# OpenMatchmaking/microservice-matchmaking

Measured on NVIDIA H100. Metric: matches/sec, higher is better.
Workload: dtype int32/u64

## Files before the change

microservice-matchmaking_b200/csrc/mm_common.cuh:

```cuda
#pragma once
#include <cuda_runtime.h>
#include <stdint.h>

#include "../../include/mm_engine.h"

namespace mm {

constexpr int kBlock = 512;
constexpr uint32_t kTile = 2048;
constexpr uint32_t kMaxRows = 2048;
constexpr uint32_t kMaxStages = 4;
constexpr uint32_t kTileBytes = kTile * (8 + 2);
constexpr uint32_t kMaxSegs = MM_MAX_GROUPS * MM_MAX_MODES;
constexpr uint32_t kChunkHist = 256;
constexpr uint32_t kFastBins = 255;
constexpr uint64_t kEmptyKey = 0xFFFFFFFFFFFFFFFFull;
constexpr uint64_t kTombKey = 0xFFFFFFFFFFFFFFFEull;
constexpr uint64_t kFreeVal = 0xFFFFFFFFFFFFFFFFull;
constexpr uint64_t kPending = 0x8000000000000000ull;
constexpr uint32_t kGenMask = 0x7FFFFFFFu;

struct PoolView {
  uint64_t* id;
  int32_t* rating;
  uint8_t* mode;
  uint8_t* tsize;
  uint32_t* ts;
  uint16_t* bin;
  uint32_t* seq;
};
struct PoolMeta {
  uint32_t* fill;
  uint32_t* chunk_tab;
  uint32_t* bump;
  uint32_t* tot;
  uint32_t* chist;
  uint32_t max_ch;
};

struct BinMap {
  const uint16_t* lut;
  int32_t key_lo;
  uint32_t KR;
  uint32_t stride;
  uint32_t K;
};

struct SegInfo {
  uint32_t n;
  uint32_t n_lobbies;
  uint32_t member_base;
  uint32_t lobby_base;
  uint32_t left_base;
  uint32_t new_chunk;
  uint32_t n_left;
  uint32_t reserved;
};

struct TickCtr {
  uint32_t gbar;
  uint32_t done;
  uint32_t n_lobbies, n_matched, n_alive, n_dead, n_resid;
  uint32_t n_tiles;
  uint32_t heavy;
  uint32_t chist_bad;
  unsigned long long t[12];
};

struct Geo {
  uint32_t T0[kMaxSegs + 1];
  uint32_t NT, tpr, n_segs, max_rows;
};

struct ActiveView {
  unsigned long long* kv;
  uint64_t mask;
  uint64_t dcap;
  __device__ __forceinline__ bool on() const { return mask != 0 || dcap != 0; }
  __device__ __forceinline__ unsigned long long* key(uint64_t h) const { return kv + 2 * h; }
  __device__ __forceinline__ unsigned long long* val(uint64_t h) const { return dcap ? kv + h : kv + 2 * h + 1; }
};

__device__ __forceinline__ uint64_t hash64(uint64_t x) {
  x ^= x >> 33; x *= 0xFF51AFD7ED558CCDull; x ^= x >> 33; x *= 0xC4CEB9FE1A85EC53ull; x ^= x >> 33;
  return x;
}
__device__ __forceinline__ uint64_t act_find(const ActiveView& a, uint64_t pid) {
  if (a.dcap) return pid < a.dcap ? pid : ~0ull;
  if (pid >= kTombKey) return ~0ull;
  uint64_t h = hash64(pid) & a.mask;
  for (uint64_t probe = 0; probe <= a.mask; ++probe) {
    const unsigned long long k = *a.key(h);
    if (k == pid) return h;
    if (k == kEmptyKey) return ~0ull;
    h = (h + 1) & a.mask;
  }
  return ~0ull;
}

__device__ __forceinline__ uint64_t policy_evict_first() {
  uint64_t p;
  asm volatile("createpolicy.fractional.L2::evict_first.b64 %0, 1.0;" : "=l"(p));
  return p;
}
__device__ __forceinline__ uint64_t policy_evict_last() {
  uint64_t p;
  asm volatile("createpolicy.fractional.L2::evict_last.b64 %0, 1.0;" : "=l"(p));
  return p;
}
__device__ __forceinline__ void st_hint_u64(uint64_t* a, uint64_t v, uint64_t pol) {
  asm volatile("st.global.L2::cache_hint.u64 [%0], %1, %2;" ::"l"(a), "l"(v), "l"(pol) : "memory");
}

__device__ __forceinline__ uint32_t smem_u32(const void* p) { return (uint32_t)__cvta_generic_to_shared(p); }
__device__ __forceinline__ void mbar_init(uint64_t* bar, uint32_t count) {
  asm volatile("mbarrier.init.shared::cta.b64 [%0], %1;" ::"r"(smem_u32(bar)), "r"(count) : "memory");
}
__device__ __forceinline__ void mbar_fence_init() { asm volatile("fence.mbarrier_init.release.cluster;" ::: "memory"); }
__device__ __forceinline__ void mbar_expect_tx(uint64_t* bar, uint32_t bytes) {
// ... 169 lines not shown
```

microservice-matchmaking_b200/csrc/mm_engine.cu:

```cuda
#include <cuda_runtime.h>

#include <algorithm>
#include <cstdio>
#include <cstdlib>
#include <cstring>
#include <mutex>
#include <new>
#include <vector>

#include "mm_kernels.cuh"

using namespace mm;

namespace {

struct Pool {
  PoolView v{};
  PoolMeta m{};
  uint32_t n = 0;
};

struct Table {
  unsigned long long* kv = nullptr;
};

}

struct mm_engine {
  mm_config cfg{};
  std::mutex mu;
  int device = 0;
  int n_sms = 0;
  size_t smem_optin = 0, smem_sm = 0;
  cudaStream_t stream = nullptr;
  bool own_stream = true;
  cudaStream_t copy_stream = nullptr;
  cudaEvent_t ev_copy = nullptr;
  cudaStream_t d2h_stream = nullptr;
  bool async_results = false, results_pending = false;
  bool last_packed = false;
  cudaEvent_t ev[5]{};
  char last_err[512] = {0};

  int32_t key_lo = 0;
  uint32_t KR = 0, stride = 0, K = 0, Kp = 0;
  uint32_t n_segs = 0;
  uint32_t n_cut = 0;
  uint16_t* d_part_cut = nullptr;
  uint32_t* d_cut_lp_lo = nullptr;
  uint16_t* d_lut = nullptr;
  uint8_t* d_grp_lut = nullptr;
  uint8_t* d_mode_tsize = nullptr;
  uint32_t* d_seg_bin_lo = nullptr;
  uint32_t* d_seg_L = nullptr;
  uint16_t* d_bin_seg = nullptr;
  uint32_t min_L = 1;
  uint32_t max_nb = 1;

  uint32_t capacity = 0;
  uint32_t n_chunks = 0;
  Pool pool[2];
  int cur = 0;
  uint32_t gen = 1;
  uint32_t seq_next = 0;
  Pool snap;
  uint32_t snap_gen = 0, snap_seq = 0;
  bool has_snap = false;

  bool use_active = true, dense_ids = false;
  uint64_t hcap = 0;
  Table tab[2];
  int tcur = 0;
  uint64_t n_active = 0, n_tomb = 0;

  uint32_t R = 0;
  uint32_t helpers = 0;
  int rows_per_sm = 2;
  int rank_impl = 3;
  uint32_t place_stages = 0;
  int fused_ok = 0;
  int tick_impl = 1;
  size_t tick_smem = 0;
  uint32_t *d_M = nullptr, *d_P = nullptr;
  uint32_t *d_outbase = nullptr, *d_binlim = nullptr;
  uint16_t* d_bin_key = nullptr;
// ... 436 lines not shown
  const uint32_t rows = tick_rows(e);
  k_place<512><<<rows, 512, place_smem_bytes(e->max_nb, e->place_stages), e->stream>>>(place_args(e, want_seq),
                                                                                  e->pool[e->cur].m.fill, e->n_segs);
  CK(cudaEventRecord(e->ev[3], e->stream));
  if (e->pool[e->cur ^ 1].m.chist)
    CK(cudaMemsetAsync(e->pool[e->cur ^ 1].m.chist, 0, (size_t)e->n_chunks * kChunkHist * 4, e->stream));
  k_epilogue<512><<<std::max<uint32_t>(1, std::min<uint32_t>((uint32_t)e->n_sms, 2 * rows)), 512, 0, e->stream>>>(epi_args(e, want_seq, true));
  CK(cudaGetLastError());
  CK(cudaEventRecord(e->ev[4], e->stream));
  CK(cudaMemcpyAsync(e->h_ctr, e->d_ctr, sizeof(TickCtr), cudaMemcpyDeviceToHost, e->stream));
  CK(cudaStreamSynchronize(e->stream));
  return MM_OK;
}

bool use_fused(const mm_engine* e) { return e->tick_impl == 1 && e->fused_ok; }

int tick_fused(mm_engine* e, bool want_seq) {
  TickArgs a{};
  const uint32_t rows = tick_rows(e);
  const uint32_t helpers = rows >= 64 ? std::min(32u, e->helpers + (e->R - rows)) : (rows > 1 ? 1u : 0u);
  a.src = e->pool[e->cur].v;
  a.R = rows;
  a.M = e->d_M;
  a.P = e->d_P;
  e->ctr_idx ^= 1;
  e->d_ctr = e->d_ctr2 + e->ctr_idx;
  a.tail = tail_args(e);
  a.place = place_args(e, want_seq);
  a.epi = epi_args(e, want_seq, want_seq || helpers == 0);
  a.next_ctr = e->d_ctr2 + (e->ctr_idx ^ 1);
  CK(cudaEventRecord(e->ev[0], e->stream));
  void* params[] = {&a};
  CK(cudaLaunchCooperativeKernel((const void*)k_tick<512>, dim3(rows + helpers), dim3(512), params, e->tick_smem, e->stream));
  CK(cudaEventRecord(e->ev[4], e->stream));
  CK(cudaMemcpyAsync(e->h_ctr, e->d_ctr, sizeof(TickCtr), cudaMemcpyDeviceToHost, e->stream));
  CK(cudaStreamSynchronize(e->stream));
  return MM_OK;
}

int tick_commit(mm_engine* e, uint32_t n, mm_tick_stats* stats) {
  const TickCtr& c = *e->h_ctr;
  mm_tick_stats st{};
  st.pool_before = n; st.n_lobbies = c.n_lobbies; st.n_matched = c.n_matched; st.n_residual = c.n_resid;
  st.n_dead = c.n_dead; st.n_launches = 4;
  float ms = 0;
  CK(cudaEventElapsedTime(&ms, e->ev[0], e->ev[4]));
  st.device_us = ms * 1000.f;
  if (e->last_fused) {
    st.n_launches = 1;
    st.hist_us = (float)(c.t[1] - c.t[0]) * 1e-3f;
    st.scan_us = (float)(c.t[2] - c.t[1]) * 1e-3f;
    st.place_us = (float)(c.t[3] - c.t[2]) * 1e-3f;
    st.epilogue_us = (float)(c.t[6] - c.t[3]) * 1e-3f;
    if (std::getenv("MM_TRACE"))
      std::fprintf(stderr, "[mm] t0=0 rows_p1_done=%.1f tail_done=%.1f bar1=%.1f place_start=%.1f rows_place_done=%.1f bar2=%.1f end=%.1f us\n",
                   (c.t[8] - c.t[0]) * 1e-3, (c.t[5] - c.t[0]) * 1e-3, (c.t[1] - c.t[0]) * 1e-3, (c.t[2] - c.t[0]) * 1e-3,
                   (c.t[10] - c.t[0]) * 1e-3, (c.t[3] - c.t[0]) * 1e-3, (c.t[6] - c.t[0]) * 1e-3);
  } else {
    CK(cudaEventElapsedTime(&ms, e->ev[0], e->ev[1]));
    st.hist_us = ms * 1000.f;
    CK(cudaEventElapsedTime(&ms, e->ev[1], e->ev[2]));
    st.scan_us = ms * 1000.f;
    CK(cudaEventElapsedTime(&ms, e->ev[2], e->ev[3]));
    st.place_us = ms * 1000.f;
    CK(cudaEventElapsedTime(&ms, e->ev[3], e->ev[4]));
    st.epilogue_us = ms * 1000.f;
  }
  e->gen = next_gen(e);
  e->cur ^= 1;
  e->pool[e->cur].n = c.n_resid;
  e->last = st;
  if (stats) *stats = st;
  if (c.chist_bad) {
    std::snprintf(e->last_err, sizeof(e->last_err), "%u placement tiles disagree with their chunk histograms", c.chist_bad);
    return MM_E_STATE;
  }
  return MM_OK;
}

int wait_results(mm_engine* e) {
  if (e->results_pending) {
    CK(cudaStreamSynchronize(e->d2h_stream));
    e->results_pending = false;
  }
  return MM_OK;
}

int tick_to_host(mm_engine* e, mm_lobby_hdr* lobbies, uint32_t lobby_cap, uint64_t* member_ids, uint32_t* member_handles,
                 uint64_t member_cap, uint32_t* emit_seq, mm_tick_stats* stats) {
  const uint32_t n = e->pool[e->cur].n;
  const bool want_members = member_ids || member_handles;
  int rc;
  const bool defer = e->async_results && e->results_pending && member_handles && !member_ids && !emit_seq &&
                     e->last_packed && e->d_hdr_alt && e->d_members32_alt;
  if (defer) {
    std::swap(e->d_hdr, e->d_hdr_alt);
    std::swap(e->d_members32, e->d_members32_alt);
  } else if ((rc = wait_results(e))) {
    return rc;
  }
  e->last_fused = use_fused(e) && (!lobbies || (uint64_t)lobby_cap >= n / e->min_L) && (!want_members || member_cap >= n);
  if (e->last_fused) {
    if ((rc = tick_fused(e, emit_seq != nullptr))) return rc;
  } else {
    if ((rc = tick_phase_a(e))) return rc;
    CK(cudaMemcpyAsync(e->h_ctr, e->d_ctr, sizeof(TickCtr), cudaMemcpyDeviceToHost, e->stream));
    CK(cudaStreamSynchronize(e->stream));
    if ((lobbies && e->h_ctr->n_lobbies > lobby_cap) || (want_members && e->h_ctr->n_matched > member_cap)) {
      std::snprintf(e->last_err, sizeof(e->last_err), "need lobby_cap >= %u, member_cap >= %u", e->h_ctr->n_lobbies,
                    e->h_ctr->n_matched);
// ... 41 lines not shown
    case MM_E_STATE: return "invalid state for this call";
    default: return "unknown status";
  }
}

const char* mm_last_error(mm_engine* e) { return e ? e->last_err : ""; }

void mm_config_default(mm_config* c) {
  if (!c) return;
  std::memset(c, 0, sizeof(*c));
  c->abi_version = MM_ABI_VERSION;
  static const int32_t lo[7] = {0, 1500, 2000, 2500, 3000, 3500, 4000};
  static const int32_t hi[7] = {1499, 1999, 2499, 2999, 3499, 3999, 5000};
  c->n_groups = 7;
  for (int g = 0; g < 7; ++g) { c->group_lo[g] = lo[g]; c->group_hi[g] = hi[g]; }
  c->default_group = 7 / 2 + 1;
  c->n_modes = 2;
  c->modes[0].teams = 2; c->modes[0].team_size = 1;
  c->modes[1].teams = 2; c->modes[1].team_size = 5;
  c->order_mode = MM_ORDER_ARRIVAL;
  c->capacity = 1u << 20;
  c->active_capacity = 0;
  c->device = 0;
  c->flags = 0;
}

int mm_group_of(const mm_config* cfg, int32_t rating) {
  if (!cfg || cfg->n_groups == 0 || cfg->n_groups > MM_MAX_GROUPS) return MM_E_ARG;
  return group_of(cfg, rating);
}

int mm_create(const mm_config* cfg, mm_engine** out) {
  if (!out) return MM_E_ARG;
  *out = nullptr;
  int rc = check_config(cfg);
  if (rc) return rc;
  int ndev = 0;
  if (cudaGetDeviceCount(&ndev) != cudaSuccess || ndev == 0 || cfg->device < 0 || cfg->device >= ndev) {
    cudaGetLastError();
    return MM_E_CUDA;
  }
  mm_engine* e = new (std::nothrow) mm_engine();
  if (!e) return MM_E_CAP;
  e->cfg = *cfg;
  e->device = cfg->device;
  e->capacity = cfg->capacity;
  e->use_active = !(cfg->flags & MM_F_NO_DEDUPE);
  e->dense_ids = e->use_active && (cfg->flags & MM_F_DENSE_IDS);
  auto bail = [&](int code) { mm_destroy(e); return code; };
  if (cudaSetDevice(e->device) != cudaSuccess) return bail(MM_E_CUDA);
  cudaDeviceProp prop{};
  if (cudaGetDeviceProperties(&prop, e->device) != cudaSuccess) return bail(MM_E_CUDA);
  e->n_sms = prop.multiProcessorCount;
  e->smem_optin = prop.sharedMemPerBlockOptin;
  e->smem_sm = prop.sharedMemPerMultiprocessor;
  if (cudaStreamCreateWithFlags(&e->stream, cudaStreamNonBlocking) != cudaSuccess) return bail(MM_E_CUDA);
  if (cudaStreamCreateWithFlags(&e->d2h_stream, cudaStreamNonBlocking) != cudaSuccess) return bail(MM_E_CUDA);
  if (cudaStreamCreateWithFlags(&e->copy_stream, cudaStreamNonBlocking) != cudaSuccess ||
      cudaEventCreateWithFlags(&e->ev_copy, cudaEventDisableTiming) != cudaSuccess)
    return bail(MM_E_CUDA);
  for (auto& ev : e->ev)
    if (cudaEventCreate(&ev) != cudaSuccess) return bail(MM_E_CUDA);
  if ((rc = build_tables(e))) return bail(rc);
  {
    const size_t static_smem = sizeof(Geo) + 512;
    const uint32_t st_max = 2;
    for (uint32_t st = st_max; st >= 2 && !e->place_stages; --st)
      if (2 * (place_smem_bytes(e->max_nb, st) + static_smem + 1024) <= e->smem_sm) { e->place_stages = st; e->rows_per_sm = 2; }
    for (uint32_t st = kMaxStages; st >= 1 && !e->place_stages; --st)
      if (place_smem_bytes(e->max_nb, st) + static_smem + 1024 <= e->smem_optin) { e->place_stages = st; e->rows_per_sm = 1; }
    if (!e->place_stages || colscan_smem(e) + static_smem + 1024 > e->smem_optin) {
      std::snprintf(e->last_err, sizeof(e->last_err), "key domain too large for shared memory: %u bins", e->Kp);
      return bail(MM_E_ARG);
    }
    bool ok = allow_max_smem(e, k_colscan) == cudaSuccess && allow_max_smem(e, k_hist<512>) == cudaSuccess &&
              allow_max_smem(e, k_place<512>) == cudaSuccess && allow_max_smem(e, k_tick<512>) == cudaSuccess;
    if (!ok) return bail(fail(e, cudaGetLastError(), "cudaFuncSetAttribute"));
  }
  e->n_chunks = (e->capacity + kTile - 1) / kTile + e->n_segs + 2;
  if ((uint64_t)e->n_chunks * e->n_segs * 4 > (8ull << 30)) return bail(MM_E_CAP);
  if ((rc = alloc_pool(e, e->pool[0])) || (rc = alloc_pool(e, e->pool[1]))) return bail(rc);
  if (cudaMalloc(&e->d_left_bits, (pool_slots(e) / 32 + 64) * 4) != cudaSuccess) return bail(MM_E_CUDA);
  if (e->use_active) {
    const uint64_t want = cfg->active_capacity ? cfg->active_capacity : 2ull * cfg->capacity;
    if (e->dense_ids) {
      e->hcap = want;
      for (auto& t : e->tab) t.kv = nullptr;
      if (cudaMalloc(&e->tab[0].kv, e->hcap * 8) != cudaSuccess) return bail(MM_E_CUDA);
    } else {
      uint64_t h = 1024;
      while (h * 3 < want * 4 + 64) h <<= 1;
      e->hcap = h;
      for (auto& t : e->tab)
        if (cudaMalloc(&t.kv, h * 16) != cudaSuccess) return bail(MM_E_CUDA);
    }
    if ((rc = clear_table(e, e->tab[0]))) return bail(rc);
  }
  const size_t cap = (size_t)e->capacity + 64;
  e->max_lobbies = e->capacity / e->min_L + 1;
  auto A = [&](void** p, size_t bytes) { return cudaMalloc(p, bytes) == cudaSuccess; };
  if (!A((void**)&e->d_outbase, (e->Kp + 1) * 4) ||
      !A((void**)&e->d_binlim, (e->Kp + 1) * 4) || !A((void**)&e->d_seg, e->n_segs * sizeof(SegInfo)) ||
      !A((void**)&e->d_members, cap * 8) || !A((void**)&e->d_src_idx, cap * 4) ||
      !A((void**)&e->d_hdr, (size_t)e->max_lobbies * sizeof(mm_lobby_hdr)) ||
      !A((void**)&e->d_emit_seq, (size_t)e->max_lobbies * 4) || !A((void**)&e->d_ctr2, 2 * sizeof(TickCtr)) ||
      !A((void**)&e->d_small, 64) ||
// ... 472 lines not shown
```

microservice-matchmaking_b200/csrc/mm_epilogue.cuh:

```cuda
#pragma once
#include "mm_common.cuh"
#include "mm_scan.cuh"

namespace mm {

constexpr uint32_t kLeftList = 2048;
constexpr uint32_t kEpiScratchWords = (kMaxRows + 1) + 64 + (kMaxSegs + 1) + 4 * kMaxSegs + kLeftList;

struct EpiArgs {
  PoolView src, dst;
  PoolMeta src_meta, dst_meta;
  uint32_t R, new_gen, n_segs, n_groups, Kp, write_headers;
  const uint32_t* rescnt;
  const uint32_t* left_bits;
  ActiveView act;
  const SegInfo* seg;
  const uint32_t* seg_L;
  const uint16_t* part_cut;
  const uint32_t* seg_bin_lo;
  mm_lobby_hdr* hdr;
  const uint32_t* src_idx;
  uint32_t* emit_seq;
  TickCtr* ctr;
};

template <int BLOCK>
__device__ __forceinline__ void headers_body(const Geo& g, const EpiArgs& a, const uint32_t* s_lbase, const uint32_t* s_mbase,
                                             const uint32_t* s_L, uint32_t part, uint32_t nparts) {
  const uint32_t tid = threadIdx.x, n_segs = a.n_segs, n_groups = a.n_groups;
  const PoolMeta sm = a.src_meta;
  const uint32_t total_lob = __ldcg(&a.ctr->n_lobbies);
  for (uint32_t sg = 0; sg < n_segs; ++sg) {
    const uint32_t l0 = s_lbase[sg], l1 = sg + 1 < n_segs ? s_lbase[sg + 1] : total_lob;
    const uint32_t L = s_L[sg], mb = s_mbase[sg];
    mm_lobby_hdr h;
    h.n_members = (uint16_t)L;
    const uint32_t cut = a.part_cut[sg];
    h.mode = (uint8_t)(cut / n_groups);
    h.group = (uint8_t)(cut % n_groups);
    for (uint32_t c = l0 + part * BLOCK + tid; c < l1; c += nparts * BLOCK) {
      h.first_member = mb + (c - l0) * L;
      a.hdr[c] = h;
      if (a.emit_seq) {
        const uint32_t v = __ldcg(&a.src_idx[h.first_member + L - 1]), p = geo_seg_of(g, v / kTile);
        a.emit_seq[c] = a.src.seq[__ldcg(&sm.chunk_tab[(size_t)p * sm.max_ch + (v / kTile - g.T0[p])]) * kTile + v % kTile];
      }
    }
  }
}
template <int BLOCK>
__device__ __forceinline__ void headers_only(uint32_t* scratch, const Geo& g, const EpiArgs& a, uint32_t part, uint32_t nparts) {
  uint32_t* s_lbase = scratch;
  uint32_t* s_mbase = s_lbase + kMaxSegs + 1;
  uint32_t* s_L = s_mbase + kMaxSegs;
  for (uint32_t s = threadIdx.x; s < a.n_segs; s += BLOCK) {
    s_lbase[s] = __ldcg(&a.seg[s].lobby_base); s_mbase[s] = __ldcg(&a.seg[s].member_base); s_L[s] = a.seg_L[s];
  }
  __syncthreads();
  headers_body<BLOCK>(g, a, s_lbase, s_mbase, s_L, part, nparts);
}

template <int BLOCK>
__device__ __forceinline__ void epilogue_body(uint32_t* scratch, const Geo& g, const EpiArgs a,
                                              unsigned long long* t_mid = nullptr) {
  const PoolView& src = a.src;
  const PoolView& dst = a.dst;
  const uint32_t R = a.R, n_segs = a.n_segs;
  const uint32_t* __restrict__ rescnt = a.rescnt;
  const uint32_t* __restrict__ left_bits = a.left_bits;
  const ActiveView act = a.act;
  const SegInfo* __restrict__ seg = a.seg;
  const uint32_t* __restrict__ seg_L = a.seg_L;
  TickCtr* ctr = a.ctr;
  const uint32_t new_gen = a.new_gen;
  const uint32_t n = g.NT * kTile;
  const uint32_t chunk = g.tpr * kTile;
  constexpr uint32_t NW = BLOCK / 32;
  const PoolMeta sm = a.src_meta;
  auto phys_of = [&](uint32_t v, uint32_t& p) -> uint32_t {
    p = geo_seg_of(g, v / kTile);
    return __ldcg(&sm.chunk_tab[(size_t)p * sm.max_ch + (v / kTile - g.T0[p])]) * kTile + v % kTile;
  };
  uint32_t* s_off = scratch;
  uint32_t* s_tmp = s_off + kMaxRows + 1;
  uint32_t* s_lbase = s_tmp + 64;
  uint32_t* s_mbase = s_lbase + kMaxSegs + 1;
  uint32_t* s_L = s_mbase + kMaxSegs;
  uint32_t* s_leftb = s_L + kMaxSegs;
  uint32_t* s_newch = s_leftb + kMaxSegs;
  uint32_t* s_list = s_newch + kMaxSegs;
  const uint32_t tid = threadIdx.x, lane = tid & 31, warp = tid >> 5;
  for (uint32_t s = tid; s < n_segs; s += BLOCK) {
    s_lbase[s] = __ldcg(&seg[s].lobby_base); s_mbase[s] = __ldcg(&seg[s].member_base); s_L[s] = seg_L[s];
    s_leftb[s] = __ldcg(&seg[s].left_base); s_newch[s] = __ldcg(&seg[s].new_chunk);
  }
  for (uint32_t r = tid; r < R; r += BLOCK) s_off[r] = __ldcg(&rescnt[r]);
  __syncthreads();
  const uint32_t total = block_excl_scan<BLOCK>(s_off, R, s_tmp);
  if (tid == 0) {
    s_off[R] = total;
    if (blockIdx.x == 0) ctr->n_resid = total;
  }
  __syncthreads();
  if (a.write_headers)
    headers_body<BLOCK>(g, a, s_lbase, s_mbase, s_L, blockIdx.x, gridDim.x);
  const uint32_t per = (total + gridDim.x - 1) / gridDim.x;
  const uint32_t r0 = (uint64_t)blockIdx.x * per < total ? blockIdx.x * per : total;
  const uint32_t r1 = r0 + per < total ? r0 + per : total;
  if (r1 > r0) {
    uint32_t tbase = r0, fill = 0;
    uint32_t row_beg = 0;
    auto flush = [&](uint32_t count, bool last) {
// ... 99 lines not shown
```

microservice-matchmaking_b200/csrc/mm_kernels.cuh:

```cuda
#pragma once
#include "mm_common.cuh"
#include "mm_hist.cuh"
#include "mm_scan.cuh"
#include "mm_place.cuh"
#include "mm_epilogue.cuh"
#include "mm_active.cuh"

namespace mm {

template <int BLOCK>
__global__ void __launch_bounds__(BLOCK, 2)
    k_hist(const uint16_t* __restrict__ bins16, const PoolMeta meta, uint32_t n_segs, uint32_t R, uint32_t Kp, uint32_t max_nb,
           const uint32_t* __restrict__ seg_bin_lo, uint32_t* __restrict__ M) {
  extern __shared__ __align__(128) unsigned char smem_raw[];
  __shared__ Geo geo;
  __shared__ uint32_t s_gtmp[33];
  geo_build<BLOCK>(geo, meta.fill, n_segs, R, s_gtmp);
  if (meta.chist) rowsum_body<BLOCK>(smem_raw, geo, meta, Kp, seg_bin_lo, M);
  else hist_body<BLOCK>(smem_raw, geo, bins16, meta, Kp, max_nb, seg_bin_lo, M);
}

struct TickArgs {
  PoolView src;
  uint32_t R;
// ... 12 lines not shown
  __shared__ Geo geo;
  __shared__ uint32_t s_gtmp[33];
  uint32_t* scratch = reinterpret_cast<uint32_t*>(smem_raw);
  const unsigned int G = gridDim.x;
  const uint32_t R = a.R, Kp = a.tail.Kp, K = a.tail.K;
  const bool is_row = blockIdx.x < R;
  const uint32_t helper = blockIdx.x - R, n_helpers = G - R;
  TickCtr* ctr = a.tail.ctr;
  unsigned int bar = 0;
  auto stamp = [&](int k) {
    if (blockIdx.x == 0 && threadIdx.x == 0) {
      unsigned long long t;
      asm volatile("mov.u64 %0, %%globaltimer;" : "=l"(t));
      ctr->t[k] = t;
    }
  };
  stamp(0);
  const bool tail_cta = blockIdx.x == G - 1;
  auto run_tail = [&]() {
    colscan_tail_body(scratch, a.tail);
    if (threadIdx.x == 0) {
      unsigned long long t;
      asm volatile("mov.u64 %0, %%globaltimer;" : "=l"(t));
      ctr->t[5] = t;
    }
  };
  const bool tail_first = tail_cta && !is_row;
  if (tail_first) {
    run_tail();
    grid_arrive(&ctr->gbar);
  }
  geo_build<BLOCK>(geo, a.place.meta.fill, a.tail.n_segs, R, s_gtmp);
  if (is_row) {
    if (a.place.meta.chist) rowsum_body<BLOCK>(smem_raw, geo, a.place.meta, Kp, a.tail.seg_bin_lo, a.M);
    else hist_body<BLOCK>(smem_raw, geo, a.src.bin, a.place.meta, Kp, a.place.max_nb, a.tail.seg_bin_lo, a.M);
  }
  if (tail_cta && is_row) run_tail();
  if (threadIdx.x == 0) { unsigned long long tm; asm volatile("mov.u64 %0, %%globaltimer;" : "=l"(tm)); if (is_row) atomicMax(&ctr->t[8], tm); }
  bar += G;
  if (tail_first) grid_wait(&ctr->gbar, bar); else grid_barrier(&ctr->gbar, bar);
  stamp(1);
  if (geo_use_colscan(geo)) {
    for (uint32_t grp = blockIdx.x; grp < (K + 31) / 32; grp += G) colscan_cols_body(scratch, geo, grp, Kp, K, a.tail.bin_seg, a.M, a.P);
    grid_barrier(&ctr->gbar, (bar += G));
  }
  stamp(2);
  if (is_row) place_body<BLOCK>(smem_raw, geo, a.place);
  if (threadIdx.x == 0 && is_row) { unsigned long long tm; asm volatile("mov.u64 %0, %%globaltimer;" : "=l"(tm)); atomicMax(&ctr->t[10], tm); }
  if (a.epi.dst_meta.chist && (!is_row || n_helpers == 0)) {
    const uint32_t part = n_helpers ? helper : blockIdx.x, nparts = n_helpers ? n_helpers : G;
    const size_t words = (size_t)__ldcg(a.epi.dst_meta.bump) * kChunkHist;
    for (size_t i = (size_t)part * BLOCK + threadIdx.x; i < words; i += (size_t)nparts * BLOCK) a.epi.dst_meta.chist[i] = 0;
  }
  if (!is_row && !a.epi.write_headers) headers_only<BLOCK>(scratch, geo, a.epi, helper, n_helpers);
  grid_barrier(&ctr->gbar, (bar += G));
  stamp(3);
  epilogue_body<BLOCK>(scratch, geo, a.epi, &ctr->t[7]);
  stamp(4);
  if (threadIdx.x == 0) {
    unsigned long long tm;
    asm volatile("mov.u64 %0, %%globaltimer;" : "=l"(tm));
    atomicMax(&ctr->t[6], tm);
    __threadfence();
    if (atomicAdd(&ctr->done, 1u) == G - 1) {
      TickCtr* nx = a.next_ctr;
      nx->gbar = 0; nx->done = 0; nx->chist_bad = 0;
      nx->t[6] = 0; nx->t[7] = 0; nx->t[8] = 0; nx->t[10] = 0;
    }
  }
}

}
```

microservice-matchmaking_b200/csrc/mm_place.cuh:

```cuda
#pragma once
#include "mm_common.cuh"

namespace mm {

constexpr uint32_t kHeadSlots = 4096;
constexpr uint32_t NW16 = 16;
constexpr uint32_t kPlaceUnionBytes = NW16 * 256 * 4 + NW16 * 256 * 2 + 1024 + kTile * 4;

__host__ __device__ constexpr uint32_t place_cnt_cap(uint32_t max_nb) { return (max_nb > 1024u ? max_nb : 1024u); }
constexpr uint32_t kHalfWarps = 8;
constexpr uint32_t kHalfBytes = kHalfWarps * 256 * 4 + kHalfWarps * 256 * 2 + 256 * 4 + kTile * 4;
__host__ __device__ constexpr size_t place_smem_whole(uint32_t max_nb, uint32_t stages) {
  return (size_t)stages * kTileBytes + 128 + (size_t)((place_cnt_cap(max_nb) + 3) & ~3u) * 4 + kPlaceUnionBytes + sizeof(DescCache) + 16;
}
__host__ __device__ constexpr size_t place_smem_halves(uint32_t max_nb, uint32_t stages) {
  return (size_t)stages * (kTileBytes + kChunkHist * 4) + 256 + (size_t)((place_cnt_cap(max_nb) + 3) & ~3u) * 4 +
         2 * kHalfBytes + sizeof(DescCache) + 16;
}
__host__ __device__ constexpr size_t place_smem_bytes(uint32_t max_nb, uint32_t stages) {
  return max_nb <= kFastBins && place_smem_halves(max_nb, stages) > place_smem_whole(max_nb, stages)
             ? place_smem_halves(max_nb, stages)
             : place_smem_whole(max_nb, stages);
}

struct PlaceArgs {
  const uint16_t* bins16;
  const uint64_t* ids;
  PoolMeta meta;
  uint32_t K, Kp, R, stages, fast_ok, max_nb;
  const uint32_t* seg_bin_lo;
  const uint16_t* bin_seg;
  const uint32_t* M;
  const uint32_t* P;
  const uint32_t* outbase;
  const uint32_t* binlim;
  uint64_t* members;
  uint32_t* src_idx;
  uint32_t* left_bits;
  uint32_t* rescnt;
  TickCtr* ctr;
};

template <int BLOCK>
__device__ __forceinline__ void place_halves(unsigned char* smem_raw, const Geo& g, const PlaceArgs a) {
  static_assert(BLOCK == 512 && kTile == 2048, "tile arrangement is written for 2 x 256 threads x 8 players");
  constexpr int J = 8;
  const uint32_t S = a.stages;
  uint64_t* ring_ids = reinterpret_cast<uint64_t*>(smem_raw);
  uint16_t* ring_bins = reinterpret_cast<uint16_t*>(smem_raw + (size_t)S * kTile * 8);
  uint32_t* ring_hist = reinterpret_cast<uint32_t*>(smem_raw + (size_t)S * kTileBytes);
  unsigned char* hdr = smem_raw + (size_t)S * (kTileBytes + kChunkHist * 4);
  uint64_t* full = reinterpret_cast<uint64_t*>(hdr);
  uint64_t* empty = full + kMaxStages;
  uint64_t* hand = empty + kMaxStages;
  uint32_t* s_nv = reinterpret_cast<uint32_t*>(hand + 1);
  uint32_t* s_b0 = s_nv + kMaxStages;
  uint32_t* s_b1 = s_b0 + kMaxStages;
  uint32_t* s_sg = s_b1 + kMaxStages;
  uint32_t* s_misc = s_sg + kMaxStages;
  uint32_t* s_wt = s_misc + 8;
  uint32_t* cnt = reinterpret_cast<uint32_t*>(hdr + 256);
  const uint32_t cnt_cap = place_cnt_cap(a.max_nb);
  unsigned char* halves = reinterpret_cast<unsigned char*>(cnt + ((cnt_cap + 3) & ~3u));
  DescCache& dc = *reinterpret_cast<DescCache*>(halves + 2 * kHalfBytes);

  const uint32_t tid = threadIdx.x, lane = tid & 31, h = tid >> 8, ht = tid & 255, hw = ht >> 5;
  const uint32_t lt_mask = (1u << lane) - 1u;
  uint32_t* wmask = reinterpret_cast<uint32_t*>(halves + h * kHalfBytes);
  uint16_t* wcnt = reinterpret_cast<uint16_t*>(wmask + kHalfWarps * 256);
  uint32_t* lgd = reinterpret_cast<uint32_t*>(wcnt + kHalfWarps * 256);
  uint32_t* spd = lgd + 256;
  const uint32_t row = blockIdx.x;
  const uint64_t pol_in = policy_evict_first();

  const uint32_t s0 = row * g.tpr < g.NT ? row * g.tpr : g.NT;
  const uint32_t s1 = s0 + g.tpr < g.NT ? s0 + g.tpr : g.NT;
  const uint32_t n_tiles = s1 - s0;

  auto issue = [&](uint32_t stage, uint32_t t) {
    uint32_t phys, nvsg;
    if (t < kDescCap) { phys = dc.phys[t]; nvsg = dc.nvsg[t]; }
    else { const TileDesc d = geo_tile(g, a.meta, s0 + t); phys = d.phys; nvsg = d.nvalid | (d.seg << 16); }
    s_nv[stage] = nvsg & 0xFFFFu;
    s_sg[stage] = nvsg >> 16;
    s_b0[stage] = a.seg_bin_lo[nvsg >> 16];
    s_b1[stage] = a.seg_bin_lo[(nvsg >> 16) + 1];
    mbar_expect_tx(&full[stage], kTileBytes + kChunkHist * 4);
    tma_load_1d(ring_ids + (size_t)stage * kTile, a.ids + (size_t)phys * kTile, kTile * 8, &full[stage], pol_in);
    tma_load_1d(ring_bins + (size_t)stage * kTile, a.bins16 + (size_t)phys * kTile, kTile * 2, &full[stage], pol_in);
    tma_load_1d(ring_hist + (size_t)stage * kChunkHist, a.meta.chist + (size_t)phys * kChunkHist, kChunkHist * 4,
                &full[stage], pol_in);
  };

  if (tid == 0) {
    for (uint32_t s = 0; s < S; ++s) { mbar_init(&full[s], 1); mbar_init(&empty[s], 256); }
    mbar_init(hand, 256);
    mbar_fence_init();
    for (uint32_t i = 0; i < 8; ++i) s_misc[i] = 0;
  }
  fence_proxy_async();
  desc_fill<BLOCK>(dc, g, a.meta, s0, s1);
  for (uint32_t i = tid; i < 2 * (kHalfWarps * 256 * 6 / 4); i += BLOCK) {
    const uint32_t hh = i / (kHalfWarps * 256 * 6 / 4), k = i % (kHalfWarps * 256 * 6 / 4);
    reinterpret_cast<uint32_t*>(halves + hh * kHalfBytes)[k] = 0;
  }
  __syncthreads();
  if (tid == 0)
    for (uint32_t t = 0; t < S && t < n_tiles; ++t) issue(t, t);

  uint32_t nleft = 0;
  const uint32_t row_p_last = n_tiles ? geo_seg_of(g, s1 - 1) : 0u;
  const bool scanned = geo_use_colscan(g);
  for (uint32_t t = h; t < n_tiles; t += 2) {
    const uint32_t st = t % S, parity = (t / S) & 1u;
    const uint32_t vbase = (s0 + t) * kTile;
    const uint16_t* tb = ring_bins + (size_t)st * kTile;
    const uint64_t* ti = ring_ids + (size_t)st * kTile;
    if (t) mbar_wait(hand, (t - 1) & 1u);
    mbar_wait(&full[st], parity);
    const uint32_t valid = s_nv[st];
    const uint32_t bin0 = s_b0[st], nb = s_b1[st] - bin0;
    const uint32_t d = ht;
    const uint32_t ch = d < nb ? ring_hist[st * kChunkHist + d] : 0u;
    const uint32_t lim = ch ? __ldcg(&a.binlim[bin0 + d]) : 0u;
    uint32_t wb = s_misc[1], we = s_misc[2];
    if (bin0 < wb || bin0 + nb > we) {
      wb = bin0; we = bin0 + nb;
      for (uint32_t p = s_sg[st] + 1; p <= row_p_last; ++p) {
        const uint32_t e = a.seg_bin_lo[p + 1];
        if (e - wb > cnt_cap) break;
        we = e;
      }
      for (uint32_t i = wb + ht; i < we; i += 256) {
        uint32_t rlo = 0, rhi = 0, v = 0;
        if (geo_rows_of(g, a.bin_seg[i], rlo, rhi) && row >= rlo && row <= rhi) {
          uint32_t pre = 0;
          if (scanned) pre = __ldcg(&a.P[(size_t)row * a.Kp + i]);
          else
            for (uint32_t r = rlo; r < row; r += 8) {
              uint32_t v8[8];
#pragma unroll
              for (uint32_t u = 0; u < 8; ++u) v8[u] = r + u < row ? __ldcg(&a.M[(size_t)(r + u) * a.Kp + i]) : 0u;
#pragma unroll
              for (uint32_t u = 0; u < 8; ++u) pre += v8[u];
            }
          v = __ldcg(&a.outbase[i]) + pre;
        }
        cnt[i - wb] = v;
      }
      bar_sync_half(h);
      if (ht == 0) { s_misc[1] = wb; s_misc[2] = we; }
    }
    uint32_t base = 0;
    if (d < nb) { base = cnt[bin0 - wb + d]; cnt[bin0 - wb + d] = base + ch; }
    mbar_arrive(hand);

    uint32_t incl = ch;
#pragma unroll
    for (int off = 1; off < 32; off <<= 1) {
      const uint32_t u = __shfl_up_sync(0xFFFFFFFFu, incl, off);
      if (lane >= (uint32_t)off) incl += u;
    }
    if (lane == 31) s_wt[h * 8 + hw] = incl;

    uint32_t pk[J];
    {
      uint32_t* wm = wmask + hw * 256;
      uint16_t* wc = wcnt + hw * 256;
      uint32_t dg[J];
#pragma unroll
      for (int j = 0; j < J; ++j) {
        const uint32_t pos = hw * (32 * J) + j * 32 + lane;
// ... 60 lines not shown
    const uint32_t tf = s_misc[3 + h];
    uint32_t lmask = 0;
    if (!(tf & 2u)) {
#pragma unroll
      for (int j = 0; j < J; ++j) {
        const uint32_t dj = pk[j] & 0xFFu;
        if (dj < nb) {
          const uint32_t pos = hw * (32 * J) + j * 32 + lane;
          const uint32_t lpos = wcnt[hw * 256 + dj] + (pk[j] >> 8);
          bool matched = true;
          if ((tf & 1u) || a.src_idx) {
            const uint32_t e = lgd[dj];
            const uint32_t slot = (e + lpos) & 0x7FFFFFFFu;
            if (e >> 31) matched = slot < __ldcg(&a.binlim[bin0 + dj]);
            if (matched && a.src_idx) a.src_idx[slot] = vbase + pos;
          }
          spd[lpos] = pos | ((matched ? dj : 255u) << 11);
          if (!matched) lmask |= 1u << j;
        }
      }
    }
    {
      uint32_t mine = 0, all = 0;
      if (tf & 1u) {
#pragma unroll
        for (int j = 0; j < J; ++j) {
          const uint32_t wv = __ballot_sync(0xFFFFFFFFu, (lmask >> j) & 1u);
          if (lane == (uint32_t)j) mine = wv;
          all += __popc(wv);
        }
      }
      if (lane < (uint32_t)J) a.left_bits[(vbase >> 5) + hw * J + lane] = mine;
      if (lane == 0) nleft += all;
    }
    __syncwarp();
    reinterpret_cast<uint4*>(wcnt + hw * 256)[lane] = make_uint4(0, 0, 0, 0);
    bar_sync_half(h);
    if (ht == 0) {
      s_misc[3 + h] = 0;
      if (tf & 2u) atomicAdd(&a.ctr->chist_bad, 1u);
    }
    if (!(tf & 2u)) {
#pragma unroll
      for (int i = 0; i < J; ++i) {
        const uint32_t k = i * 256 + ht;
        if (k < n_live) {
          const uint32_t v = spd[k], dk = v >> 11;
          if (dk != 255u) a.members[(lgd[dk] + k) & 0x7FFFFFFFu] = ti[v & 0x7FFu];
        }
      }
    }
    mbar_arrive(&empty[st]);
    if (ht == 0 && t + S < n_tiles) {
      mbar_wait(&empty[st], parity);
      issue(st, t + S);
    }
  }

  if (lane == 0 && nleft) atomicAdd(&s_misc[0], nleft);
  __syncthreads();
  if (tid == 0) {
    a.rescnt[row] = s_misc[0];
    for (uint32_t s = 0; s < S; ++s) { mbar_inval(&full[s]); mbar_inval(&empty[s]); }
    mbar_inval(hand);
  }
}

template <int BLOCK>
__device__ __forceinline__ void place_body(unsigned char* smem_raw, const Geo& g, const PlaceArgs a) {
  static_assert(BLOCK == 512 && kTile == 2048, "tile arrangement is written for 512 threads x 4 players");
  if (a.meta.chist && a.fast_ok) {
    place_halves<BLOCK>(smem_raw, g, a);
    return;
  }
  constexpr int J = kTile / BLOCK;
  constexpr int NW = BLOCK / 32;
  const uint32_t stages = a.stages, K = a.K, Kp = a.Kp;
  uint64_t* ring_ids = reinterpret_cast<uint64_t*>(smem_raw);
  uint16_t* ring_bins = reinterpret_cast<uint16_t*>(smem_raw + (size_t)stages * kTile * 8);
  uint64_t* full = reinterpret_cast<uint64_t*>(smem_raw + (size_t)stages * kTileBytes);
  uint32_t* s_nv = reinterpret_cast<uint32_t*>(smem_raw + (size_t)stages * kTileBytes + 32);
  uint32_t* s_sg = s_nv + kMaxStages;
  uint32_t* s_b0 = s_sg + kMaxStages;
  uint32_t* s_b1 = s_b0 + kMaxStages;
  uint32_t* s_misc = s_b1 + kMaxStages;
  uint32_t* cnt = reinterpret_cast<uint32_t*>(smem_raw + (size_t)stages * kTileBytes + 128);
  const uint32_t cnt_cap = place_cnt_cap(a.max_nb);
  unsigned char* uni = reinterpret_cast<unsigned char*>(cnt + ((cnt_cap + 3) & ~3u));
  DescCache& dc = *reinterpret_cast<DescCache*>(uni + kPlaceUnionBytes);
  uint32_t* head = reinterpret_cast<uint32_t*>(uni);
  uint32_t* node = head + kHeadSlots;
  uint16_t* nbin = reinterpret_cast<uint16_t*>(node + kTile);
  uint32_t* wmask = reinterpret_cast<uint32_t*>(uni);
  uint16_t* wcnt = reinterpret_cast<uint16_t*>(wmask + NW * 256);
  uint32_t* wcnt32 = reinterpret_cast<uint32_t*>(wcnt);
  uint32_t* lgd = wcnt32 + NW * 128;
  uint32_t* spd = lgd + 256;

  const uint32_t tid = threadIdx.x, lane = tid & 31, warp = tid >> 5;
  const uint32_t lt_mask = (1u << lane) - 1u;
  const uint32_t row = blockIdx.x;
  const uint64_t pol_in = policy_evict_first();

  const uint32_t s0 = row * g.tpr < g.NT ? row * g.tpr : g.NT;
  const uint32_t s1 = s0 + g.tpr < g.NT ? s0 + g.tpr : g.NT;
  const uint32_t n_tiles = s1 - s0;

  uint32_t dbase = 0;
  auto issue = [&](uint32_t stage, uint32_t t) {
// ... 345 lines not shown
```

Measured before the change: 5.701 billion.

## Write lobby headers on row blocks via atomic chunk claiming; add place stall counters

The standalone header pass moves from helper blocks with a fixed partition to row blocks that claim 8192-lobby chunks through an atomic counter. Each lobby then finds its segment by binary search over segment lobby bases, which balances the header work across blocks before the grid barrier. The change also adds clock()-based stall counters in the placement pipeline, accumulated into TickCtr and printed under MM_TRACE. Those counters add a few clock reads and shared-memory updates per tile, plus global atomics per row.

```diff
diff --git a/microservice-matchmaking_b200/csrc/mm_common.cuh b/microservice-matchmaking_b200/csrc/mm_common.cuh
--- a/microservice-matchmaking_b200/csrc/mm_common.cuh
+++ b/microservice-matchmaking_b200/csrc/mm_common.cuh
@@ -64,7 +64,9 @@
   uint32_t n_tiles;
   uint32_t heavy;
   uint32_t chist_bad;
+  uint32_t hdr_next;
   unsigned long long t[12];
+  unsigned long long stall[2][4];
 };
 
 struct Geo {
diff --git a/microservice-matchmaking_b200/csrc/mm_engine.cu b/microservice-matchmaking_b200/csrc/mm_engine.cu
--- a/microservice-matchmaking_b200/csrc/mm_engine.cu
+++ b/microservice-matchmaking_b200/csrc/mm_engine.cu
@@ -31,6 +31,7 @@
   std::mutex mu;
   int device = 0;
   int n_sms = 0;
+  int clock_khz = 0;
   size_t smem_optin = 0, smem_sm = 0;
   cudaStream_t stream = nullptr;
   bool own_stream = true;
@@ -573,10 +574,15 @@
     st.scan_us = (float)(c.t[2] - c.t[1]) * 1e-3f;
     st.place_us = (float)(c.t[3] - c.t[2]) * 1e-3f;
     st.epilogue_us = (float)(c.t[6] - c.t[3]) * 1e-3f;
-    if (std::getenv("MM_TRACE"))
-      std::fprintf(stderr, "[mm] t0=0 rows_p1_done=%.1f tail_done=%.1f bar1=%.1f place_start=%.1f rows_place_done=%.1f bar2=%.1f end=%.1f us\n",
+    if (std::getenv("MM_TRACE")) {
+      const double us = 1e3 / ((double)e->clock_khz * tick_rows(e));
+      std::fprintf(stderr, "[mm] t0=0 rows_p1_done=%.1f tail_done=%.1f bar1=%.1f place_start=%.1f rows_place_done=%.1f bar2=%.1f end=%.1f us"
+                   " | place stall/row hand full empty loop: h0 %.1f %.1f %.1f %.1f h1 %.1f %.1f %.1f %.1f us\n",
                    (c.t[8] - c.t[0]) * 1e-3, (c.t[5] - c.t[0]) * 1e-3, (c.t[1] - c.t[0]) * 1e-3, (c.t[2] - c.t[0]) * 1e-3,
-                   (c.t[10] - c.t[0]) * 1e-3, (c.t[3] - c.t[0]) * 1e-3, (c.t[6] - c.t[0]) * 1e-3);
+                   (c.t[10] - c.t[0]) * 1e-3, (c.t[3] - c.t[0]) * 1e-3, (c.t[6] - c.t[0]) * 1e-3,
+                   c.stall[0][0] * us, c.stall[0][1] * us, c.stall[0][2] * us, c.stall[0][3] * us,
+                   c.stall[1][0] * us, c.stall[1][1] * us, c.stall[1][2] * us, c.stall[1][3] * us);
+    }
   } else {
     CK(cudaEventElapsedTime(&ms, e->ev[0], e->ev[1]));
     st.hist_us = ms * 1000.f;
@@ -724,6 +730,7 @@
   cudaDeviceProp prop{};
   if (cudaGetDeviceProperties(&prop, e->device) != cudaSuccess) return bail(MM_E_CUDA);
   e->n_sms = prop.multiProcessorCount;
+  if (cudaDeviceGetAttribute(&e->clock_khz, cudaDevAttrClockRate, e->device) != cudaSuccess) return bail(MM_E_CUDA);
   e->smem_optin = prop.sharedMemPerBlockOptin;
   e->smem_sm = prop.sharedMemPerMultiprocessor;
   if (cudaStreamCreateWithFlags(&e->stream, cudaStreamNonBlocking) != cudaSuccess) return bail(MM_E_CUDA);
diff --git a/microservice-matchmaking_b200/csrc/mm_epilogue.cuh b/microservice-matchmaking_b200/csrc/mm_epilogue.cuh
--- a/microservice-matchmaking_b200/csrc/mm_epilogue.cuh
+++ b/microservice-matchmaking_b200/csrc/mm_epilogue.cuh
@@ -48,16 +48,37 @@
     }
   }
 }
-template <int BLOCK>
-__device__ __forceinline__ void headers_only(uint32_t* scratch, const Geo& g, const EpiArgs& a, uint32_t part, uint32_t nparts) {
+constexpr uint32_t kHdrChunk = 8192;
+template <int BLOCK>
+__device__ __forceinline__ void headers_claimed(uint32_t* scratch, const EpiArgs& a, uint32_t* next) {
   uint32_t* s_lbase = scratch;
   uint32_t* s_mbase = s_lbase + kMaxSegs + 1;
   uint32_t* s_L = s_mbase + kMaxSegs;
-  for (uint32_t s = threadIdx.x; s < a.n_segs; s += BLOCK) {
+  uint32_t* s_claim = s_L + kMaxSegs;
+  const uint32_t tid = threadIdx.x, n_segs = a.n_segs, n_groups = a.n_groups;
+  const uint32_t total_lob = __ldcg(&a.ctr->n_lobbies);
+  for (uint32_t s = tid; s < n_segs; s += BLOCK) {
     s_lbase[s] = __ldcg(&a.seg[s].lobby_base); s_mbase[s] = __ldcg(&a.seg[s].member_base); s_L[s] = a.seg_L[s];
   }
-  __syncthreads();
-  headers_body<BLOCK>(g, a, s_lbase, s_mbase, s_L, part, nparts);
+  for (;;) {
+    if (tid == 0) *s_claim = atomicAdd(next, 1u);
+    __syncthreads();
+    const uint32_t c0 = *s_claim * kHdrChunk;
+    __syncthreads();
+    if (c0 >= total_lob) break;
+    const uint32_t c1 = c0 + kHdrChunk < total_lob ? c0 + kHdrChunk : total_lob;
+    for (uint32_t c = c0 + tid; c < c1; c += BLOCK) {
+      uint32_t lo = 0, hi = n_segs;
+      while (hi - lo > 1) { const uint32_t mid = (lo + hi) >> 1; if (s_lbase[mid] <= c) lo = mid; else hi = mid; }
+      mm_lobby_hdr h;
+      h.n_members = (uint16_t)s_L[lo];
+      const uint32_t cut = a.part_cut[lo];
+      h.mode = (uint8_t)(cut / n_groups);
+      h.group = (uint8_t)(cut % n_groups);
+      h.first_member = s_mbase[lo] + (c - s_lbase[lo]) * s_L[lo];
+      a.hdr[c] = h;
+    }
+  }
 }
 
 template <int BLOCK>
diff --git a/microservice-matchmaking_b200/csrc/mm_kernels.cuh b/microservice-matchmaking_b200/csrc/mm_kernels.cuh
--- a/microservice-matchmaking_b200/csrc/mm_kernels.cuh
+++ b/microservice-matchmaking_b200/csrc/mm_kernels.cuh
@@ -88,7 +88,7 @@
     const size_t words = (size_t)__ldcg(a.epi.dst_meta.bump) * kChunkHist;
     for (size_t i = (size_t)part * BLOCK + threadIdx.x; i < words; i += (size_t)nparts * BLOCK) a.epi.dst_meta.chist[i] = 0;
   }
-  if (!is_row && !a.epi.write_headers) headers_only<BLOCK>(scratch, geo, a.epi, helper, n_helpers);
+  if (is_row && !a.epi.write_headers) headers_claimed<BLOCK>(scratch, a.epi, &ctr->hdr_next);
   grid_barrier(&ctr->gbar, (bar += G));
   stamp(3);
   epilogue_body<BLOCK>(scratch, geo, a.epi, &ctr->t[7]);
@@ -100,8 +100,9 @@
     __threadfence();
     if (atomicAdd(&ctr->done, 1u) == G - 1) {
       TickCtr* nx = a.next_ctr;
-      nx->gbar = 0; nx->done = 0; nx->chist_bad = 0;
+      nx->gbar = 0; nx->done = 0; nx->chist_bad = 0; nx->hdr_next = 0;
       nx->t[6] = 0; nx->t[7] = 0; nx->t[8] = 0; nx->t[10] = 0;
+      for (int i = 0; i < 8; ++i) nx->stall[i / 4][i % 4] = 0;
     }
   }
 }
diff --git a/microservice-matchmaking_b200/csrc/mm_place.cuh b/microservice-matchmaking_b200/csrc/mm_place.cuh
--- a/microservice-matchmaking_b200/csrc/mm_place.cuh
+++ b/microservice-matchmaking_b200/csrc/mm_place.cuh
@@ -10,11 +10,12 @@
 __host__ __device__ constexpr uint32_t place_cnt_cap(uint32_t max_nb) { return (max_nb > 1024u ? max_nb : 1024u); }
 constexpr uint32_t kHalfWarps = 8;
 constexpr uint32_t kHalfBytes = kHalfWarps * 256 * 4 + kHalfWarps * 256 * 2 + 256 * 4 + kTile * 4;
+constexpr uint32_t kHalvesHdr = 288;
 __host__ __device__ constexpr size_t place_smem_whole(uint32_t max_nb, uint32_t stages) {
   return (size_t)stages * kTileBytes + 128 + (size_t)((place_cnt_cap(max_nb) + 3) & ~3u) * 4 + kPlaceUnionBytes + sizeof(DescCache) + 16;
 }
 __host__ __device__ constexpr size_t place_smem_halves(uint32_t max_nb, uint32_t stages) {
-  return (size_t)stages * (kTileBytes + kChunkHist * 4) + 256 + (size_t)((place_cnt_cap(max_nb) + 3) & ~3u) * 4 +
+  return (size_t)stages * (kTileBytes + kChunkHist * 4) + kHalvesHdr + (size_t)((place_cnt_cap(max_nb) + 3) & ~3u) * 4 +
          2 * kHalfBytes + sizeof(DescCache) + 16;
 }
 __host__ __device__ constexpr size_t place_smem_bytes(uint32_t max_nb, uint32_t stages) {
@@ -59,7 +60,8 @@
   uint32_t* s_sg = s_b1 + kMaxStages;
   uint32_t* s_misc = s_sg + kMaxStages;
   uint32_t* s_wt = s_misc + 8;
-  uint32_t* cnt = reinterpret_cast<uint32_t*>(hdr + 256);
+  uint32_t* s_ck = s_wt + 16;
+  uint32_t* cnt = reinterpret_cast<uint32_t*>(hdr + kHalvesHdr);
   const uint32_t cnt_cap = place_cnt_cap(a.max_nb);
   unsigned char* halves = reinterpret_cast<unsigned char*>(cnt + ((cnt_cap + 3) & ~3u));
   DescCache& dc = *reinterpret_cast<DescCache*>(halves + 2 * kHalfBytes);
@@ -96,7 +98,7 @@
     for (uint32_t s = 0; s < S; ++s) { mbar_init(&full[s], 1); mbar_init(&empty[s], 256); }
     mbar_init(hand, 256);
     mbar_fence_init();
-    for (uint32_t i = 0; i < 8; ++i) s_misc[i] = 0;
+    for (uint32_t i = 0; i < 8; ++i) { s_misc[i] = 0; s_ck[i] = 0; }
   }
   fence_proxy_async();
   desc_fill<BLOCK>(dc, g, a.meta, s0, s1);
@@ -111,13 +113,18 @@
   uint32_t nleft = 0;
   const uint32_t row_p_last = n_tiles ? geo_seg_of(g, s1 - 1) : 0u;
   const bool scanned = geo_use_colscan(g);
+  uint32_t* ck = s_ck + 4 * h;
+  if (ht == 0) ck[3] = (uint32_t)clock();
   for (uint32_t t = h; t < n_tiles; t += 2) {
     const uint32_t st = t % S, parity = (t / S) & 1u;
     const uint32_t vbase = (s0 + t) * kTile;
     const uint16_t* tb = ring_bins + (size_t)st * kTile;
     const uint64_t* ti = ring_ids + (size_t)st * kTile;
+    const uint32_t ck0 = (uint32_t)clock();
     if (t) mbar_wait(hand, (t - 1) & 1u);
+    const uint32_t ck1 = (uint32_t)clock();
     mbar_wait(&full[st], parity);
+    if (ht == 0) { ck[0] += ck1 - ck0; ck[1] += (uint32_t)clock() - ck1; }
     const uint32_t valid = s_nv[st];
     const uint32_t bin0 = s_b0[st], nb = s_b1[st] - bin0;
     const uint32_t d = ht;
@@ -284,9 +291,15 @@
     }
     mbar_arrive(&empty[st]);
     if (ht == 0 && t + S < n_tiles) {
+      const uint32_t ck2 = (uint32_t)clock();
       mbar_wait(&empty[st], parity);
+      ck[2] += (uint32_t)clock() - ck2;
       issue(st, t + S);
     }
+  }
+  if (ht == 0) {
+    ck[3] = (uint32_t)clock() - ck[3];
+    for (uint32_t k = 0; k < 4; ++k) atomicAdd(&a.ctr->stall[h][k], (unsigned long long)ck[k]);
   }
 
   if (lane == 0 && nleft) atomicAdd(&s_misc[0], nleft);
```

New measurement: 6.534 billion, median of 6. 1.15x the previous value.
